# Kamino666/video_features

Hardware: AMD Instinct MI355X
Metric: frames/sec CLIP-ViT-B/32 uni_12 (higher is better)
Workload: dtype bf16; 1 GPU; model=CLIP-ViT-B/32, global_batch=256, seq_len=12, resolution=224, parallelism=dp1

## Files before the change

video_features_amd/models/clip_vit.py:

```python
from __future__ import annotations

from dataclasses import dataclass
from typing import Optional

import torch
import torch.nn.functional as F
from torch import nn

from .. import ops


@dataclass
class ViTConfig:
    input_resolution: int = 224
    patch_size: int = 32
    width: int = 768
    layers: int = 12
    heads: int = 12
    output_dim: int = 512


VIT_B32 = ViTConfig(patch_size=32)
VIT_B16 = ViTConfig(patch_size=16)

# ... 60 lines not shown
            ops.fused_ln_tiles(x, self.attn.proj.weight)
            and ops.fused_ln_tiles(x, self.mlp.c_fc.weight))

    def attn_mlp_folded(self, y1: torch.Tensor, s1: torch.Tensor):
        proj, fc, ln = self.attn.proj, self.mlp.c_fc, self.ln_2
        s2, st2 = ops.linear_res_stats(self.attn.heads_out(y1), proj.weight,
                                       proj.bias, s1)
        h = ops.linear_ln_act(
            s2, st2, *self._ln2_fold(), act='quick_gelu', eps=ln.eps,
            unfolded=(fc.weight, fc.bias, ln.weight, ln.bias))
        return self.mlp.c_proj(h), s2


class VisionTransformer(nn.Module):
    def __init__(self, cfg: ViTConfig = VIT_B32):
        super().__init__()
        self.cfg = cfg
        w = cfg.width
        self.conv1 = nn.Conv2d(3, w, kernel_size=cfg.patch_size,
                               stride=cfg.patch_size, bias=False)
        n_patches = (cfg.input_resolution // cfg.patch_size) ** 2
        scale = w ** -0.5
        self.class_embedding = nn.Parameter(scale * torch.randn(w))
        self.positional_embedding = nn.Parameter(
            scale * torch.randn(n_patches + 1, w))
        self.ln_pre = LayerNorm(w)
        self.blocks = nn.ModuleList(
            [ResidualAttentionBlock(w, cfg.heads) for _ in range(cfg.layers)])
        self.ln_post = LayerNorm(w)
        self.proj = nn.Parameter(scale * torch.randn(w, cfg.output_dim))

    def _patch_embed(self, x: torch.Tensor) -> torch.Tensor:
        if x.is_cuda:
            t = x.shape[0]
            p = self.cfg.patch_size
            g = x.shape[-1] // p
            xp = x.reshape(t, 3, g, p, g, p).permute(0, 2, 4, 1, 3, 5)
            xp = xp.reshape(t, g * g, 3 * p * p)
            w = self.conv1.weight.reshape(self.cfg.width, -1)
            return xp @ w.t()
        x = self.conv1(x)
        return x.flatten(2).transpose(1, 2)

    def forward(self, x: torch.Tensor) -> torch.Tensor:
        x = self._patch_embed(x)
        x = ops.clip_embed_ln(x, self.class_embedding,
                              self.positional_embedding, self.ln_pre.weight,
                              self.ln_pre.bias, self.ln_pre.eps)
        full_tail = ops._env_flag('VFA_CLIP_FULL_TAIL')
        delta, res = None, x
        for blk in (self.blocks if full_tail else self.blocks[:-1]):
            if delta is None:
                y1, s1 = blk.ln_1(res), res
            else:
                y1, s1 = ops.layer_norm_residual(delta, res, blk.ln_1.weight,
                                                 blk.ln_1.bias, blk.ln_1.eps)
            if blk.fold_routed(s1):
                delta, res = blk.attn_mlp_folded(y1, s1)
                continue
            a = blk.attn(y1)
            y2, s2 = ops.layer_norm_residual(a, s1, blk.ln_2.weight,
                                             blk.ln_2.bias, blk.ln_2.eps)
            delta, res = blk.mlp(y2), s2
        if full_tail:
            x = delta + res
            x = self.ln_post(x[:, 0, :])
        else:
            x = self._cls_tail(self.blocks[-1], delta, res)
        return x @ self.proj.to(x.dtype)

    def _cls_tail(self, blk: ResidualAttentionBlock,
# ... 31 lines not shown
```

video_features_amd/ops/__init__.py:

```python
from __future__ import annotations

import math
import os
from typing import Optional

import torch

_ext = None
_ext_err: Optional[str] = None


def _env_flag(name: str) -> bool:
    return os.environ.get(name, '').strip().lower() not in (
        '', '0', 'false', 'no', 'off')


def _load_extension():
    global _ext, _ext_err
    if _ext is not None or _ext_err is not None:
        return _ext
    try:
        from . import _vfa_hip
        _ext = _vfa_hip
    except ImportError as e:
# ... 95 lines not shown
        y, s = _ext.layer_norm_residual(x.contiguous(), res.contiguous(),
                                        weight, bias, eps)
        return y, s
    s = x + res
    y = torch.nn.functional.layer_norm(s, (s.shape[-1],), weight, bias, eps)
    return y, s


def clip_embed_ln(pe: torch.Tensor, cls: torch.Tensor, pos: torch.Tensor,
                  weight: torch.Tensor, bias: torch.Tensor,
                  eps: float = 1e-5) -> torch.Tensor:
    if (_use_hip(pe) and pe.shape[-1] % 8 == 0
            and pe.dtype in _FLOAT_DTYPES):
        return _ext.clip_embed_ln(pe.contiguous(), cls, pos, weight, bias,
                                  eps)
    c = cls.to(pe.dtype).expand(pe.shape[0], 1, -1)
    x = torch.cat([c, pe], dim=1) + pos.to(pe.dtype)
    return layer_norm(x, weight, bias, eps)


def preprocess_u8_chw(frames_u8: torch.Tensor, mean, std,
                      bf16: bool = True) -> torch.Tensor:
    if _use_hip(frames_u8) and \
            (frames_u8.shape[1] * frames_u8.shape[2]) % 4 == 0:
        return _ext.u8_chw_norm(frames_u8.contiguous(), list(map(float, mean)),
                                list(map(float, std)), bf16)
    x = frames_u8.permute(0, 3, 1, 2).float() / 255.0
    mean_t = torch.as_tensor(mean, dtype=x.dtype, device=x.device)
    std_t = torch.as_tensor(std, dtype=x.dtype, device=x.device)
    x = (x - mean_t[:, None, None]) / std_t[:, None, None]
    return x.to(torch.bfloat16) if bf16 else x


def mhsa_fused(qkv: torch.Tensor, heads: int,
               scale: Optional[float] = None) -> torch.Tensor:
    b, n, three_e = qkv.shape
    e = three_e // 3
    d = e // heads
    if scale is None:
        scale = 1.0 / math.sqrt(d)
    if _use_hip(qkv) and qkv.dtype == torch.bfloat16 and d == 64:
        qkv5 = qkv.view(b, n, 3, heads, d)
        return _ext.flash_qkv(qkv5.contiguous(), float(scale))
    q, k, v = qkv.view(b, n, 3, heads, d).permute(2, 0, 3, 1, 4).unbind(0)
    o = attention(q.contiguous(), k.contiguous(), v.contiguous(), scale)
    return o.permute(0, 2, 1, 3).reshape(b, n, e)


def pwc_correlation(f1: torch.Tensor, f2: torch.Tensor,
                    max_disp: int = 4, out: Optional[torch.Tensor] = None,
                    out_off: int = 0, act: str = 'none') -> torch.Tensor:
    if act not in ('none', 'leaky_relu'):
        raise ValueError(f'pwc_correlation: unsupported act {act!r}')
    leaky = act == 'leaky_relu'
    if _use_hip(f1):
        direct = out is None or (
            out.dtype == torch.bfloat16
            and out.is_contiguous(memory_format=torch.channels_last))
        if (max_disp == 4 and f1.dtype == torch.bfloat16
                and f2.dtype == torch.bfloat16 and _cl_only(f1)
                and _cl_only(f2)):
            y = _ext.pwc_correlation_nhwc(f1, f2, out if direct else None,
                                          out_off, leaky)
        else:
            y = _ext.pwc_correlation(f1.contiguous(), f2.contiguous(),
                                     max_disp, out if direct else None,
                                     out_off, leaky)
        if direct:
            return y
    else:
        y = _pwc_correlation_torch(f1, f2, max_disp)
        if leaky:
            y = torch.nn.functional.leaky_relu(y, 0.1)
    return _store_slice(out, out_off, y)


# ... 581 lines not shown
```

video_features_amd/ops/csrc/attention_flash.hip:

```cpp
#include "vfa_common.h"

typedef __bf16 bf16x8 __attribute__((ext_vector_type(8)));
typedef float f32x4 __attribute__((ext_vector_type(4)));

namespace {

constexpr int QBLK = 64;
constexpr int KVBLK = 64;
constexpr int D = 64;
constexpr int LSTR = D + 8;

__device__ __forceinline__ float group16_max(float v) {
#pragma unroll
  for (int off = 8; off > 0; off >>= 1) v = fmaxf(v, __shfl_xor(v, off, 64));
  return v;
}

__device__ __forceinline__ float group16_sum(float v) {
#pragma unroll
  for (int off = 8; off > 0; off >>= 1) v += __shfl_xor(v, off, 64);
  return v;
}

__device__ __forceinline__ void stage_rows(const __bf16* g, int rows,
// ... 137 lines not shown
      for (int r = 0; r < 4; ++r)
        p_lds[(hi4 * 4 + r) * LSTR + nt * 16 + lo] = (__bf16)p_vals[nt][r];
    asm volatile("s_waitcnt lgkmcnt(0)" ::: "memory");

#pragma unroll
    for (int kt = 0; kt < 2; ++kt) {
      bf16x8 a = *reinterpret_cast<const bf16x8*>(
          p_lds + lo * LSTR + kt * 32 + hi4 * 8);
#pragma unroll
      for (int nt = 0; nt < 4; ++nt) {
        bf16x8 bfr = *reinterpret_cast<const bf16x8*>(
            s_vt + (nt * 16 + lo) * LSTR + kt * 32 + hi4 * 8);
        o_acc[nt] =
            __builtin_amdgcn_mfma_f32_16x16x32_bf16(a, bfr, o_acc[nt], 0, 0, 0);
      }
    }
  }

#pragma unroll
  for (int r = 0; r < 4; ++r) {
    const int grow = qbase + wave * 16 + hi4 * 4 + r;
    if (grow >= n) continue;
    const float inv_l = 1.0f / l_run[r];
    __bf16* orow = out + ((long long)bi * n + grow) * (h_total * D) +
                   (long long)hi * D;
#pragma unroll
    for (int nt = 0; nt < 4; ++nt)
      orow[nt * 16 + lo] = (__bf16)(o_acc[nt][r] * inv_l);
  }
  __syncthreads();
  }
}

__global__ __launch_bounds__(256)
void flash_qkv_small_kernel(const __bf16* __restrict__ qkv,
                            __bf16* __restrict__ out,
                            int b_total, int n, int h_total, float scale) {
  extern __shared__ __attribute__((aligned(16))) char smem[];
  __bf16* s_k0 = reinterpret_cast<__bf16*>(smem);
  __bf16* s_vt0 = s_k0 + 2 * KVBLK * LSTR;
  __bf16* s_p = s_vt0 + 2 * D * LSTR;

  const int tid = threadIdx.x;
  const int lane = tid & 63, wave = tid >> 6;
  const int lo = lane & 15, hi4 = lane >> 4;
  const long long row_stride = 3LL * h_total * D;
  const int total = b_total * h_total;
  const int qr = min(wave * 16 + lo, n - 1);

  int bh = blockIdx.x;
  if (bh >= total) return;

  bf16x8 a_cur[2];
  {
    const int bi = bh / h_total, hi = bh % h_total;
    const __bf16* k_g = qkv + (long long)bi * n * row_stride +
                        ((long long)1 * h_total + hi) * D;
    stage_rows(k_g, KVBLK, row_stride, s_k0, n);
    stage_vt(k_g + (long long)h_total * D, row_stride, s_vt0, n);
    const __bf16* q_g = qkv + (long long)bi * n * row_stride +
                        (long long)hi * D;
#pragma unroll
    for (int kt = 0; kt < 2; ++kt)
      a_cur[kt] = *reinterpret_cast<const bf16x8*>(
          q_g + (long long)qr * row_stride + kt * 32 + hi4 * 8);
  }
  __syncthreads();

  int buf = 0;
  for (; bh < total; bh += gridDim.x) {
    const int nbh = bh + gridDim.x;
    const bool has_next = nbh < total;
    const int pf = has_next ? nbh : bh;
    const int pbi = pf / h_total, phi = pf % h_total;
    const __bf16* k_gn = qkv + (long long)pbi * n * row_stride +
                         ((long long)1 * h_total + phi) * D;
    const __bf16* v_gn = k_gn + (long long)h_total * D;
    uint4 kreg[2], vreg[2];
#pragma unroll
    for (int i = 0; i < 2; ++i) {
      const int t = tid + i * 256, row = t >> 3, seg = t & 7;
      kreg[i] = row < n ? *reinterpret_cast<const uint4*>(
                              k_gn + row * row_stride + seg * 8)
                        : uint4{0u, 0u, 0u, 0u};
    }
#pragma unroll
    for (int i = 0; i < 2; ++i) {
      const int t = tid + i * 256, key = t & 63, seg = t >> 6;
      vreg[i] = key < n ? *reinterpret_cast<const uint4*>(
                              v_gn + key * row_stride + seg * 8)
                        : uint4{0u, 0u, 0u, 0u};
    }
    bf16x8 a_next[2];
    {
      const __bf16* q_gn = qkv + (long long)pbi * n * row_stride +
                           (long long)phi * D;
#pragma unroll
      for (int kt = 0; kt < 2; ++kt)
        a_next[kt] = *reinterpret_cast<const bf16x8*>(
            q_gn + (long long)qr * row_stride + kt * 32 + hi4 * 8);
    }

    const __bf16* s_k = s_k0 + buf * KVBLK * LSTR;
    const __bf16* s_vt = s_vt0 + buf * D * LSTR;
    f32x4 s_frag[4];
#pragma unroll
    for (int t = 0; t < 4; ++t) s_frag[t] = f32x4{0.f, 0.f, 0.f, 0.f};
#pragma unroll
    for (int kt = 0; kt < 2; ++kt)
#pragma unroll
      for (int nt = 0; nt < 4; ++nt) {
        bf16x8 bfr = *reinterpret_cast<const bf16x8*>(
            s_k + (nt * 16 + lo) * LSTR + kt * 32 + hi4 * 8);
        s_frag[nt] = __builtin_amdgcn_mfma_f32_16x16x32_bf16(
            a_cur[kt], bfr, s_frag[nt], 0, 0, 0);
      }

    float p_vals[4][4], l_run[4];
#pragma unroll
    for (int r = 0; r < 4; ++r) {
      float mx = -1e30f;
#pragma unroll
      for (int nt = 0; nt < 4; ++nt) {
        float s = s_frag[nt][r] * scale;
        if (nt * 16 + lo >= n) s = -1e30f;
        s_frag[nt][r] = s;
        mx = fmaxf(mx, s);
      }
      mx = group16_max(mx);
      float rowsum = 0.f;
#pragma unroll
      for (int nt = 0; nt < 4; ++nt) {
        const float p = __expf(s_frag[nt][r] - mx);
        p_vals[nt][r] = p;
        rowsum += p;
      }
      l_run[r] = group16_sum(rowsum);
    }

    __bf16* p_lds = s_p + wave * 16 * LSTR;
#pragma unroll
    for (int nt = 0; nt < 4; ++nt)
#pragma unroll
      for (int r = 0; r < 4; ++r)
        p_lds[(hi4 * 4 + r) * LSTR + nt * 16 + lo] = (__bf16)p_vals[nt][r];
    asm volatile("s_waitcnt lgkmcnt(0)" ::: "memory");

    f32x4 o_acc[4];
#pragma unroll
    for (int t = 0; t < 4; ++t) o_acc[t] = f32x4{0.f, 0.f, 0.f, 0.f};
#pragma unroll
    for (int kt = 0; kt < 2; ++kt) {
      bf16x8 a = *reinterpret_cast<const bf16x8*>(
          p_lds + lo * LSTR + kt * 32 + hi4 * 8);
#pragma unroll
      for (int nt = 0; nt < 4; ++nt) {
        bf16x8 bfr = *reinterpret_cast<const bf16x8*>(
            s_vt + (nt * 16 + lo) * LSTR + kt * 32 + hi4 * 8);
        o_acc[nt] = __builtin_amdgcn_mfma_f32_16x16x32_bf16(
            a, bfr, o_acc[nt], 0, 0, 0);
      }
    }

    {
      const int bi = bh / h_total, hi = bh % h_total;
#pragma unroll
      for (int r = 0; r < 4; ++r) {
        const int grow = wave * 16 + hi4 * 4 + r;
        if (grow >= n) continue;
        const float inv_l = 1.0f / l_run[r];
        __bf16* orow = out + ((long long)bi * n + grow) * (h_total * D) +
                       (long long)hi * D;
#pragma unroll
        for (int nt = 0; nt < 4; ++nt)
          orow[nt * 16 + lo] = (__bf16)(o_acc[nt][r] * inv_l);
      }
    }

    __bf16* d_k = s_k0 + (buf ^ 1) * KVBLK * LSTR;
    __bf16* d_vt = s_vt0 + (buf ^ 1) * D * LSTR;
#pragma unroll
    for (int i = 0; i < 2; ++i) {
      const int t = tid + i * 256, row = t >> 3, seg = t & 7;
      *reinterpret_cast<uint4*>(d_k + row * LSTR + seg * 8) = kreg[i];
    }
#pragma unroll
    for (int i = 0; i < 2; ++i) {
      const int t = tid + i * 256, key = t & 63, seg = t >> 6;
      const __bf16* e = reinterpret_cast<const __bf16*>(&vreg[i]);
#pragma unroll
      for (int j = 0; j < 8; ++j) d_vt[(seg * 8 + j) * LSTR + key] = e[j];
    }
    __syncthreads();
    buf ^= 1;
    a_cur[0] = a_next[0];
    a_cur[1] = a_next[1];
  }
}

__global__ void mfma_gemm16_kernel(const float* a, const float* b, float* d) {
  const int l = threadIdx.x, lo = l & 15, hi4 = l >> 4;
  bf16x8 av, bv;
#pragma unroll
  for (int j = 0; j < 8; ++j) {
    av[j] = (__bf16)a[lo * 32 + hi4 * 8 + j];
    bv[j] = (__bf16)b[(hi4 * 8 + j) * 16 + lo];
  }
  f32x4 c = {0.f, 0.f, 0.f, 0.f};
  c = __builtin_amdgcn_mfma_f32_16x16x32_bf16(av, bv, c, 0, 0, 0);
#pragma unroll
  for (int r = 0; r < 4; ++r) d[(hi4 * 4 + r) * 16 + lo] = c[r];
}

}

extern "C" {

void vfa_flash_qkv(const void* qkv, void* out, int b, int n, int h,
                   float scale, hipStream_t stream) {
  static const bool no_pipe = [] {
    const char* e = getenv("VFA_NO_FLASHPIPE");
    return e && e[0] && e[0] != '0';
  }();
  if (n <= KVBLK && !no_pipe) {
    dim3 grid(min(b * h, 1024), 1);
    size_t lds = (size_t)(2 * (KVBLK + D) + 4 * 16) * LSTR * sizeof(__bf16);
    hipLaunchKernelGGL(flash_qkv_small_kernel, grid, dim3(256), lds, stream,
                       (const __bf16*)qkv, (__bf16*)out, b, n, h, scale);
    return;
  }
  dim3 grid(min(b * h, 2048), (n + QBLK - 1) / QBLK);
  size_t lds = (size_t)(QBLK + KVBLK + D + 4 * 16) * LSTR * sizeof(__bf16);
  hipLaunchKernelGGL(flash_qkv_kernel, grid, dim3(256), lds, stream,
                     (const __bf16*)qkv, (__bf16*)out, b, n, h, scale);
}

void vfa_mfma_gemm16(const void* a, const void* b, void* d,
                     hipStream_t stream) {
  hipLaunchKernelGGL(mfma_gemm16_kernel, dim3(1), dim3(64), 0, stream,
                     (const float*)a, (const float*)b, (float*)d);
}

}
```

video_features_amd/ops/csrc/attnpool.hip:

```cpp
#include "vfa_common.h"

namespace {

__global__ void attnpool_tokens_kernel(const uint4* __restrict__ x,
                                       const uint4* __restrict__ pos,
                                       uint4* __restrict__ t, long long b,
                                       int hw, int c8) {
  const long long total = b * c8;
  const float inv = 1.f / (float)hw;
  for (long long i = (long long)blockIdx.x * blockDim.x + threadIdx.x;
       i < total; i += (long long)gridDim.x * blockDim.x) {
    const long long bi = i / c8;
    const int ci = (int)(i % c8);
    const uint4* xb = x + bi * hw * c8 + ci;
    uint4* tb = t + bi * (hw + 1) * c8 + ci;
    float sum[8] = {0.f, 0.f, 0.f, 0.f, 0.f, 0.f, 0.f, 0.f};
    for (int j = 0; j < hw; ++j) {
      float xv[8], pv[8];
      bf16x8_to_f32(xb[(long long)j * c8], xv);
      bf16x8_to_f32(pos[(long long)(j + 1) * c8 + ci], pv);
#pragma unroll
      for (int e = 0; e < 8; ++e) {
        sum[e] += xv[e];
        xv[e] += pv[e];
      }
      tb[(long long)(j + 1) * c8] = f32_to_bf16x8(xv);
    }
    float pv[8];
    bf16x8_to_f32(pos[ci], pv);
#pragma unroll
    for (int e = 0; e < 8; ++e) sum[e] = sum[e] * inv + pv[e];
    tb[0] = f32_to_bf16x8(sum);
  }
}

__global__ __launch_bounds__(256) void attention_pool_d64_kernel(
    const __hip_bfloat16* __restrict__ q, const __hip_bfloat16* __restrict__ kv,
    __hip_bfloat16* __restrict__ out, long long bh, int heads, int l,
    float scale) {
  const int lane = threadIdx.x & 63;
  const long long pair = (long long)blockIdx.x * 4 + (threadIdx.x >> 6);
  if (pair >= bh) return;
  const long long bi = pair / heads;
  const int h = (int)(pair % heads);
  const long long c = (long long)heads * 64;
  float qf[64];
  {
    const uint4* qp = reinterpret_cast<const uint4*>(q + bi * c + h * 64);
#pragma unroll
    for (int s = 0; s < 8; ++s) {
      bf16x8_to_f32(qp[s], qf + 8 * s);
#pragma unroll
      for (int e = 0; e < 8; ++e) qf[8 * s + e] *= scale;
    }
  }
  const __hip_bfloat16* kb = kv + bi * l * 2 * c + h * 64;
  const __hip_bfloat16* vb = kb + c;
  float m = -INFINITY, denom = 0.f, acc = 0.f;
  for (int c0 = 0; c0 < l; c0 += 64) {
    const int nk = min(64, l - c0);
    const int j = c0 + lane;
    float s = -INFINITY;
    if (j < l) {
      const uint4* kp =
          reinterpret_cast<const uint4*>(kb + (long long)j * 2 * c);
      float dot = 0.f;
#pragma unroll
      for (int u = 0; u < 8; ++u) {
        float kf[8];
        bf16x8_to_f32(kp[u], kf);
#pragma unroll
        for (int e = 0; e < 8; ++e) dot += qf[8 * u + e] * kf[e];
      }
      s = dot;
    }
    const float m_new = fmaxf(m, wave_allreduce_max(s));
    const float p = (j < l) ? __expf(s - m_new) : 0.f;
    const float alpha = __expf(m - m_new);
    denom = denom * alpha + wave_allreduce_sum(p);
    acc *= alpha;
    const __hip_bfloat16* vp = vb + (long long)c0 * 2 * c + lane;
    for (int jj = 0; jj < nk; ++jj) {
      const float pj = __shfl(p, jj, 64);
      acc += pj * __bfloat162float(vp[(long long)jj * 2 * c]);
    }
    m = m_new;
  }
  out[bi * c + h * 64 + lane] = __float2bfloat16(acc / denom);
}

}

extern "C" {

void vfa_attnpool_tokens(const void* x, const void* pos, void* t, long long b,
                         int hw, int c, hipStream_t stream) {
  const long long total = b * (c / 8);
  if (total <= 0) return;
  const int grid = (int)min((total + 63) / 64, (long long)2048);
  hipLaunchKernelGGL(attnpool_tokens_kernel, dim3(grid), dim3(64), 0, stream,
                     (const uint4*)x, (const uint4*)pos, (uint4*)t, b, hw,
                     c / 8);
}

void vfa_attention_pool_d64(const void* q, const void* kv, void* out,
                            long long b, int heads, int l, float scale,
                            hipStream_t stream) {
  const long long bh = b * heads;
  if (bh <= 0) return;
  const long long grid = (bh + 3) / 4;
  hipLaunchKernelGGL(attention_pool_d64_kernel, dim3((unsigned)grid),
                     dim3(256), 0, stream, (const __hip_bfloat16*)q,
                     (const __hip_bfloat16*)kv, (__hip_bfloat16*)out, bh,
                     heads, l, scale);
}

}
```

video_features_amd/ops/csrc/bindings.cpp:

```cpp
#include <torch/extension.h>
#include <c10/hip/HIPStream.h>
#include <mutex>
#include <unordered_map>
#include <hip/hip_runtime.h>
#include <hip/hip_bf16.h>

#include "vfa_api.h"

namespace {

int dtype_tag(torch::ScalarType s) {
  switch (s) {
    case torch::kFloat32: return 0;
    case torch::kBFloat16: return 1;
    case torch::kFloat16: return 2;
    default:
      TORCH_CHECK(false, "unsupported dtype ", s);
  }
}

int dtype_tag(const torch::Tensor& t) { return dtype_tag(t.scalar_type()); }

hipStream_t current_stream() {
  return c10::hip::getCurrentHIPStream().stream();
// ... 211 lines not shown
                                               torch::Tensor b, double eps) {
  TORCH_CHECK(x.is_cuda() && x.is_contiguous() && res.is_contiguous());
  TORCH_CHECK(x.sizes() == res.sizes());
  const int d = (int)x.size(-1);
  auto wc = w.contiguous().to(x.scalar_type());
  auto bc = b.contiguous().to(x.scalar_type());
  auto y = torch::empty_like(x);
  auto s = torch::empty_like(x);
  vfa_layer_norm_residual(x.data_ptr(), res.data_ptr(), wc.data_ptr(),
                          bc.data_ptr(), y.data_ptr(), s.data_ptr(),
                          x.numel() / d, d, (float)eps, dtype_tag(x),
                          current_stream());
  return {y, s};
}

torch::Tensor u8_chw_norm(torch::Tensor frames, std::vector<double> mean,
                          std::vector<double> std_, bool bf16) {
  TORCH_CHECK(frames.is_cuda() && frames.is_contiguous());
  TORCH_CHECK(frames.scalar_type() == torch::kUInt8);
  TORCH_CHECK(frames.dim() == 4 && frames.size(3) == 3, "(T,H,W,3) expected");
  const long long t = frames.size(0);
  const int h = (int)frames.size(1), w = (int)frames.size(2);
  TORCH_CHECK((h * w) % 4 == 0);
  float m[3] = {(float)mean[0], (float)mean[1], (float)mean[2]};
  float s[3] = {(float)std_[0], (float)std_[1], (float)std_[2]};
  auto out = torch::empty({(long)t, 3, h, w},
                          frames.options().dtype(bf16 ? torch::kBFloat16
                                                      : torch::kFloat32));
  vfa_u8_chw_norm(frames.data_ptr(), out.data_ptr(), t, h, w, m, s,
                  bf16 ? 1 : 0, current_stream());
  return out;
}

torch::Tensor flash_qkv(torch::Tensor qkv, double scale) {
  TORCH_CHECK(qkv.is_cuda() && qkv.is_contiguous() && qkv.dim() == 5);
  TORCH_CHECK(qkv.size(2) == 3 && qkv.size(4) == 64,
              "flash_qkv covers head_dim 64");
  TORCH_CHECK(qkv.scalar_type() == torch::kBFloat16);
  const int b = (int)qkv.size(0), n = (int)qkv.size(1);
  const int h = (int)qkv.size(3);
  auto out = torch::empty({b, n, h * 64L}, qkv.options());
  vfa_flash_qkv(qkv.data_ptr(), out.data_ptr(), b, n, h, (float)scale,
                current_stream());
  return out;
}

torch::Tensor mfma_gemm16(torch::Tensor a, torch::Tensor b) {
  TORCH_CHECK(a.is_cuda() && a.is_contiguous() && b.is_contiguous());
  TORCH_CHECK(a.sizes() == torch::IntArrayRef({16, 32}) &&
              b.sizes() == torch::IntArrayRef({32, 16}));
  auto af = a.to(torch::kFloat32), bf = b.to(torch::kFloat32);
  auto d = torch::empty({16, 16}, af.options());
  vfa_mfma_gemm16(af.data_ptr(), bf.data_ptr(), d.data_ptr(),
                  current_stream());
  return d;
}

torch::Tensor corr_lookup(std::vector<torch::Tensor> pyramid,
                          torch::Tensor coords, bool nhwc,
                          torch::ScalarType out_dtype, bool force_gmem) {
  const int levels = (int)pyramid.size();
  TORCH_CHECK(levels >= 1 && levels <= 4, "1..4 pyramid levels");
  const int tag = dtype_tag(out_dtype);
  TORCH_CHECK(coords.is_cuda() && coords.dim() == 4 && coords.size(1) == 2);
  auto cc = coords.to(torch::kFloat32).contiguous();
  const long long b = coords.size(0);
  const int h = (int)coords.size(2), w = (int)coords.size(3);
  const long long npix = b * h * w;
  CorrPyramid pyr;
  long long lds_floats = 0;
  for (int l = 0; l < levels; ++l) {
    auto& t = pyramid[l];
    TORCH_CHECK(t.is_cuda() && t.is_contiguous() &&
                t.scalar_type() == torch::kFloat32);
    TORCH_CHECK(t.size(0) == npix && t.size(1) == 1, "plane-per-pixel");
    pyr.hs[l] = (int)t.size(2);
// ... 424 lines not shown
  auto t = torch::empty({x.size(0), hw + 1, c}, x.options());
  vfa_attnpool_tokens(x.data_ptr(), pos.data_ptr(), t.data_ptr(), x.size(0),
                      (int)hw, (int)c, current_stream());
  return t;
}

torch::Tensor attention_pool(torch::Tensor q, torch::Tensor kv,
                             int64_t heads) {
  TORCH_CHECK(q.is_cuda() && q.dim() == 2 && q.is_contiguous());
  TORCH_CHECK(kv.is_cuda() && kv.dim() == 3 && kv.is_contiguous());
  TORCH_CHECK(q.scalar_type() == torch::kBFloat16 &&
              kv.scalar_type() == torch::kBFloat16, "attention_pool: bf16");
  const int64_t b = q.size(0), c = q.size(1), l = kv.size(1);
  TORCH_CHECK(heads >= 1 && c == heads * 64,
              "attention_pool covers head_dim 64");
  TORCH_CHECK(kv.size(0) == b && kv.size(2) == 2 * c && l >= 1,
              "kv must be (B, L>=1, 2C)");
  auto out = torch::empty({b, c}, q.options());
  vfa_attention_pool_d64(q.data_ptr(), kv.data_ptr(), out.data_ptr(), b,
                         (int)heads, (int)l, 0.125f, current_stream());
  return out;
}

}

PYBIND11_MODULE(TORCH_EXTENSION_NAME, m) {
  m.def("quick_gelu", &quick_gelu);
  m.def("gelu_tanh", &gelu_tanh);
  m.def("layer_norm", &layer_norm);
  m.def("bilinear_warp", &bilinear_warp);
  m.def("grid_sample_bilinear", &grid_sample_bilinear);
  m.def("pwc_correlation", &pwc_correlation);
  m.def("mhsa", &mhsa);
  m.def("flash_qkv", &flash_qkv);
  m.def("mfma_gemm16", &mfma_gemm16);
  m.def("layer_norm_residual", &layer_norm_residual);
  m.def("clip_embed_ln", &clip_embed_ln);
  m.def("u8_chw_norm", &u8_chw_norm);
  m.def("corr_lookup", &corr_lookup);
  m.def("convex_upsample", &convex_upsample);
  m.def("gru_zr", &gru_zr);
  m.def("gru_out", &gru_out);
  m.def("instance_norm2d", &instance_norm2d);
  m.def("maxpool3d_same", &maxpool3d_same);
  m.def("maxpool2d_same", &maxpool2d_same);
  m.def("linear_act", &linear_act);
  m.def("linear_res_stats", &linear_res_stats);
  m.def("linear_ln_act", &linear_ln_act);
  m.def("conv2d_nhwc", &conv2d_nhwc);
  m.def("conv2d_tile", &conv2d_tile);
  m.def("conv_transpose2d_nhwc", &conv_transpose2d_nhwc);
  m.def("conv_transpose2d_small", &conv_transpose2d_small);
  m.def("bilinear_warp_nhwc", &bilinear_warp_nhwc);
  m.def("pwc_correlation_nhwc", &pwc_correlation_nhwc);
  m.def("temporal_merge", &temporal_merge);
  m.def("avgpool2d_nhwc", &avgpool2d_nhwc);
  m.def("attnpool_tokens", &attnpool_tokens);
  m.def("attention_pool", &attention_pool);
  m.attr("gfx_arch") = "gfx950";
}
```

video_features_amd/ops/csrc/preprocess.hip:

```cpp
#include "vfa_common.h"
#include <type_traits>

namespace {

template <typename T>
__global__ void u8_chw_norm_kernel(const unsigned char* __restrict__ in,
                                   T* __restrict__ out, long long t, int h,
                                   int w, float m0, float m1, float m2,
                                   float s0, float s1, float s2) {
  const long long hw = (long long)h * w;
  const long long quads_per_img = hw / 4;
  const long long total = t * quads_per_img;
  const float inv255 = 1.0f / 255.0f;
  const float im[3] = {m0, m1, m2};
  const float is[3] = {1.0f / s0, 1.0f / s1, 1.0f / s2};
  for (long long i = (long long)blockIdx.x * blockDim.x + threadIdx.x;
       i < total; i += (long long)gridDim.x * blockDim.x) {
    const long long ti = i / quads_per_img;
    const long long q = i % quads_per_img;
    const unsigned char* src = in + (ti * hw + q * 4) * 3;
    const uint3 raw = *reinterpret_cast<const uint3*>(src);
    unsigned char px[12];
    *reinterpret_cast<uint3*>(px) = raw;
    T planes[3][4];
#pragma unroll
    for (int p = 0; p < 4; ++p) {
#pragma unroll
      for (int c = 0; c < 3; ++c) {
        float v = (float)px[p * 3 + c] * inv255;
        planes[c][p] = from_f32<T>((v - im[c]) * is[c]);
      }
    }
    using VecElt =
        typename std::conditional<sizeof(T) == 2, unsigned short, unsigned>::type;
    using Vec = __attribute__((ext_vector_type(4))) VecElt;
#pragma unroll
    for (int c = 0; c < 3; ++c) {
      T* dst = out + (ti * 3 + c) * hw + q * 4;
      *reinterpret_cast<Vec*>(dst) = *reinterpret_cast<Vec*>(planes[c]);
    }
  }
}

}

extern "C" void vfa_u8_chw_norm(const void* in, void* out, long long t,
                                int h, int w, const float* mean,
                                const float* std, int dtype,
                                hipStream_t stream) {
  long long total = t * ((long long)h * w / 4);
  int block = 256;
  int grid = (int)min((total + block - 1) / block, (long long)4096);
  if (dtype == VFA_BF16) {
    hipLaunchKernelGGL((u8_chw_norm_kernel<__hip_bfloat16>), dim3(grid),
                       dim3(block), 0, stream, (const unsigned char*)in,
                       (__hip_bfloat16*)out, t, h, w, mean[0], mean[1],
                       mean[2], std[0], std[1], std[2]);
  } else {
    hipLaunchKernelGGL((u8_chw_norm_kernel<float>), dim3(grid), dim3(block),
                       0, stream, (const unsigned char*)in, (float*)out, t, h,
                       w, mean[0], mean[1], mean[2], std[0], std[1], std[2]);
  }
}
```

video_features_amd/ops/csrc/vfa_api.h:

```cpp
#pragma once
#include <hip/hip_runtime.h>

struct ConvGeom {
  int b, hp, wp, cin;
  int oh, ow, kout;
  int kh, kw, sh, sw;
  int pt, pl;
  int kr;
};

struct ConvAddr {
  int dh, dw;
  int ldx;
};

struct CorrPyramid {
  const void* lvl[4];
  int hs[4], ws[4];
};

struct PoolGeom {
  int in[3], out[3];
  int k[3], s[3];
  int pad[3];
// ... 21 lines not shown
void vfa_bilinear_warp(const void* x, const void* flow, void* out, int b,
                       int c, int h, int w, int dtype, hipStream_t stream);
void vfa_bilinear_warp_nhwc(const void* x, const void* flow, void* out, int b,
                            int c, int h, int w, long long fb, long long fc,
                            long long fh, long long fw, float scale,
                            hipStream_t stream);
void vfa_grid_sample(const void* x, const void* coords, void* out,
                     long long n, int c, int h, int w, int ho, int wo,
                     int dtype, hipStream_t stream);

void vfa_corr_repack(const void* in, void* out, int b, int c, int h, int w,
                     int dtype, hipStream_t stream);
void vfa_pwc_correlation(const void* f1, const void* f1p, const void* f2p,
                         void* out, int b, int c, int h, int w, int dtype,
                         int ldo, int leaky, hipStream_t stream);
void vfa_pwc_correlation_nhwc(const void* f1, const void* f2, void* out,
                              int b, int c, int h, int w, int ldo, int leaky,
                              hipStream_t stream);

long long vfa_tconv_lds_bytes(int c, int kout);
void vfa_tconv_pform(const void* x, const void* wp, const void* bias,
                     void* part, void* out, int b, int h, int w, int c,
                     int ldx, int kout, int ldo, hipStream_t stream);
void vfa_tconv_direct(const void* x, const void* wgt, const void* bias,
                      void* out, int b, int c, int h, int w, long long sb,
                      long long sc, long long sh, long long sw, int kout,
                      int ldo, hipStream_t stream);

void vfa_mhsa_small(const void* q, const void* k, const void* v, void* out,
                    int bh, int n, int d, float scale, int dtype,
                    hipStream_t stream);

void vfa_flash_qkv(const void* qkv, void* out, int b, int n, int h,
                   float scale, hipStream_t stream);
void vfa_mfma_gemm16(const void* a, const void* b, void* d,
                     hipStream_t stream);

void vfa_u8_chw_norm(const void* in, void* out, long long t, int h, int w,
                     const float* mean, const float* std, int dtype,
                     hipStream_t stream);

void vfa_corr_lookup(const CorrPyramid& pyr, const void* coords, void* out,
                     int levels, long long npix, int hw, int lds_floats,
                     int nhwc, int dtype, hipStream_t stream);
void vfa_convex_upsample(const void* flow, const void* mask, void* out, int b,
                         int h, int w, int nhwc, int dtype,
                         hipStream_t stream);
void vfa_gru_zr(const void* zr, const void* hx, void* rhx, void* z, int b,
                int c, int cx, long long hw, int nhwc, int dtype,
                hipStream_t stream);
void vfa_gru_out(const void* q, const void* z, void* hx, int b, int c, int cx,
                 long long hw, int nhwc, int dtype, hipStream_t stream);

void vfa_instance_norm2d(const void* x, void* out, int b, int c, int hw,
                         float eps, int relu, int nhwc, int dtype,
                         hipStream_t stream);

void vfa_maxpool3d_same(const void* x, void* out, long long bc,
                        const PoolGeom& g, int dtype, hipStream_t stream);
void vfa_maxpool2d_same(const void* x, void* out, long long n, int c,
                        const PoolGeom& g, int nhwc, int dtype,
                        hipStream_t stream);
void vfa_avgpool2d_nhwc(const void* x, void* out, long long n, int c, int ih,
                        int iw, int oh, int ow, int k, hipStream_t stream);

void vfa_linear_act(const void* a, const void* w, const void* bias,
                    const void* res, void* c, int m, int n, int k, int act,
                    hipStream_t stream);
void vfa_linear_res_stats(const void* a, const void* w, const void* bias,
                          const void* res, void* c, void* part, int m, int n,
                          int k, hipStream_t stream);
void vfa_linear_ln_act(const void* a, const void* stats, int groups,
                       const void* w, const void* ln_c, const void* ln_b,
// ... 24 lines not shown
```

Baseline: 87150 frames/sec.

## Rewrite small-seq flash attention with register-resident 32x32 MFMA, add patchify kernel

Replaces the block-per-head small-sequence attention kernel with a wave-per-(head, 32-query block) kernel. It keeps Q and K in registers, uses 32x32x16 MFMAs, and reads V through a transposing LDS load (ds_read_b64_tr_b16). Softmax reductions use permlane32 swaps, and the next unit's loads are prefetched in software. It also adds a dedicated vectorized patchify kernel in place of the torch permute+copy, and rewrites the attention-pool kernel to process 8 keys per wave iteration with vectorized K/V loads. The aim is to remove LDS round-trips, __syncthreads, and the extra permute copy, at the cost of more complex register-heavy code that depends on gfx950-specific instructions.

Result: faster. 90050 frames/sec, median of 6 (+3.3%).

```diff
diff --git a/video_features_amd/models/clip_vit.py b/video_features_amd/models/clip_vit.py
--- a/video_features_amd/models/clip_vit.py
+++ b/video_features_amd/models/clip_vit.py
@@ -116,11 +116,7 @@
 
     def _patch_embed(self, x: torch.Tensor) -> torch.Tensor:
         if x.is_cuda:
-            t = x.shape[0]
-            p = self.cfg.patch_size
-            g = x.shape[-1] // p
-            xp = x.reshape(t, 3, g, p, g, p).permute(0, 2, 4, 1, 3, 5)
-            xp = xp.reshape(t, g * g, 3 * p * p)
+            xp = ops.patchify(x, self.cfg.patch_size)
             w = self.conv1.weight.reshape(self.cfg.width, -1)
             return xp @ w.t()
         x = self.conv1(x)
diff --git a/video_features_amd/ops/__init__.py b/video_features_amd/ops/__init__.py
--- a/video_features_amd/ops/__init__.py
+++ b/video_features_amd/ops/__init__.py
@@ -151,8 +151,29 @@
     return x.to(torch.bfloat16) if bf16 else x
 
 
+def patchify(x: torch.Tensor, p: int) -> torch.Tensor:
+    t, c, h, w = x.shape
+    if h % p or w % p:
+        raise ValueError(f'patchify: H, W = {h}, {w} must be multiples of '
+                         f'p = {p}')
+    es = x.element_size()
+    if (_use_hip(x) and es in (2, 4) and (p * es) % 16 == 0
+            and x.numel() > 0):
+        xc = x.contiguous()
+        if xc.data_ptr() % 16 == 0:
+            return _ext.patchify(xc, int(p))
+    gy, gx = h // p, w // p
+    xp = x.reshape(t, c, gy, p, gx, p).permute(0, 2, 4, 1, 3, 5)
+    return xp.reshape(t, gy * gx, c * p * p)
+
+
+MHSA_VARIANTS = (0, 1)
+
+
 def mhsa_fused(qkv: torch.Tensor, heads: int,
-               scale: Optional[float] = None) -> torch.Tensor:
+               scale: Optional[float] = None, variant: int = 0) -> torch.Tensor:
+    if variant not in MHSA_VARIANTS:
+        raise ValueError(f'mhsa_fused: variant must be one of {MHSA_VARIANTS}')
     b, n, three_e = qkv.shape
     e = three_e // 3
     d = e // heads
@@ -160,7 +181,7 @@
         scale = 1.0 / math.sqrt(d)
     if _use_hip(qkv) and qkv.dtype == torch.bfloat16 and d == 64:
         qkv5 = qkv.view(b, n, 3, heads, d)
-        return _ext.flash_qkv(qkv5.contiguous(), float(scale))
+        return _ext.flash_qkv(qkv5.contiguous(), float(scale), int(variant))
     q, k, v = qkv.view(b, n, 3, heads, d).permute(2, 0, 3, 1, 4).unbind(0)
     o = attention(q.contiguous(), k.contiguous(), v.contiguous(), scale)
     return o.permute(0, 2, 1, 3).reshape(b, n, e)
diff --git a/video_features_amd/ops/csrc/attention_flash.hip b/video_features_amd/ops/csrc/attention_flash.hip
--- a/video_features_amd/ops/csrc/attention_flash.hip
+++ b/video_features_amd/ops/csrc/attention_flash.hip
@@ -193,169 +193,187 @@
   }
 }
 
-__global__ __launch_bounds__(256)
-void flash_qkv_small_kernel(const __bf16* __restrict__ qkv,
-                            __bf16* __restrict__ out,
-                            int b_total, int n, int h_total, float scale) {
-  extern __shared__ __attribute__((aligned(16))) char smem[];
-  __bf16* s_k0 = reinterpret_cast<__bf16*>(smem);
-  __bf16* s_vt0 = s_k0 + 2 * KVBLK * LSTR;
-  __bf16* s_p = s_vt0 + 2 * D * LSTR;
-
-  const int tid = threadIdx.x;
-  const int lane = tid & 63, wave = tid >> 6;
-  const int lo = lane & 15, hi4 = lane >> 4;
+typedef float f32x16 __attribute__((ext_vector_type(16)));
+typedef unsigned u32x2 __attribute__((ext_vector_type(2)));
+
+constexpr int RSTR = 192;
+constexpr int RIMG = 64 * RSTR;
+constexpr int RWAVES = 4;
+constexpr int RBLOCKS = 768;
+
+struct RegsLoads {
+  bf16x8 k[2][4];
+  bf16x8 q[4];
+  uint4 v[8];
+};
+
+__device__ __forceinline__ void regs_load(RegsLoads& ld,
+                                          const __bf16* __restrict__ qkv,
+                                          int u, int nqb, int n, int h_total,
+                                          int lane) {
+  const int pair = u / nqb, qb = u - pair * nqb;
+  const int bi = pair / h_total, hi = pair - bi * h_total;
   const long long row_stride = 3LL * h_total * D;
-  const int total = b_total * h_total;
-  const int qr = min(wave * 16 + lo, n - 1);
-
-  int bh = blockIdx.x;
-  if (bh >= total) return;
-
-  bf16x8 a_cur[2];
-  {
-    const int bi = bh / h_total, hi = bh % h_total;
-    const __bf16* k_g = qkv + (long long)bi * n * row_stride +
-                        ((long long)1 * h_total + hi) * D;
-    stage_rows(k_g, KVBLK, row_stride, s_k0, n);
-    stage_vt(k_g + (long long)h_total * D, row_stride, s_vt0, n);
-    const __bf16* q_g = qkv + (long long)bi * n * row_stride +
-                        (long long)hi * D;
+  const __bf16* base = qkv + (long long)bi * n * row_stride + (long long)hi * D;
+  const int r = lane & 31, h8 = (lane >> 5) * 8;
+  const __bf16* qp = base + (long long)min(qb * 32 + r, n - 1) * row_stride + h8;
+#pragma unroll
+  for (int s = 0; s < 4; ++s)
+    ld.q[s] = *reinterpret_cast<const bf16x8*>(qp + s * 16);
+#pragma unroll
+  for (int kt = 0; kt < 2; ++kt) {
+    const __bf16* kp = base + (long long)h_total * D +
+                       (long long)min(kt * 32 + r, n - 1) * row_stride + h8;
+#pragma unroll
+    for (int s = 0; s < 4; ++s)
+      ld.k[kt][s] = *reinterpret_cast<const bf16x8*>(kp + s * 16);
+  }
+  const __bf16* vp = base + 2LL * h_total * D + (lane & 7) * 8;
+#pragma unroll
+  for (int i = 0; i < 8; ++i)
+    ld.v[i] = *reinterpret_cast<const uint4*>(
+        vp + (long long)min(i * 8 + (lane >> 3), n - 1) * row_stride);
+}
+
+#define VFA_TR8(OFF)                                            \
+  asm volatile(                                                 \
+      "ds_read_b64_tr_b16 %0, %8 offset:" #OFF "+0\n\t"         \
+      "ds_read_b64_tr_b16 %1, %8 offset:" #OFF "+1536\n\t"      \
+      "ds_read_b64_tr_b16 %2, %8 offset:" #OFF "+3072\n\t"      \
+      "ds_read_b64_tr_b16 %3, %8 offset:" #OFF "+4608\n\t"      \
+      "ds_read_b64_tr_b16 %4, %8 offset:" #OFF "+6144\n\t"      \
+      "ds_read_b64_tr_b16 %5, %8 offset:" #OFF "+7680\n\t"      \
+      "ds_read_b64_tr_b16 %6, %8 offset:" #OFF "+9216\n\t"      \
+      "ds_read_b64_tr_b16 %7, %8 offset:" #OFF "+10752\n\t"     \
+      "s_waitcnt lgkmcnt(0)"                                    \
+      : "=&v"(t[0]), "=&v"(t[1]), "=&v"(t[2]), "=&v"(t[3]),     \
+        "=&v"(t[4]), "=&v"(t[5]), "=&v"(t[6]), "=&v"(t[7])      \
+      : "v"(tr_addr)                                            \
+      : "memory")
+
+__device__ __forceinline__ bf16x8 regs_join(u32x2 lo, u32x2 hi) {
+  typedef unsigned u32x4 __attribute__((ext_vector_type(4)));
+  const u32x4 v = {lo[0], lo[1], hi[0], hi[1]};
+  return __builtin_bit_cast(bf16x8, v);
+}
+
+__global__ __launch_bounds__(RWAVES * 64)
+__attribute__((amdgpu_waves_per_eu(3, 3)))
+void flash_qkv_regs_kernel(const __bf16* __restrict__ qkv,
+                           __bf16* __restrict__ out,
+                           int units, int nqb, int n, int h_total,
+                           float scale) {
+  __shared__ __attribute__((aligned(16))) char s_v[RWAVES * RIMG];
+  const int lane = threadIdx.x & 63;
+  const int wave = __builtin_amdgcn_readfirstlane(threadIdx.x >> 6);
+  const int nwaves = gridDim.x * RWAVES;
+  int u = blockIdx.x * RWAVES + wave;
+  if (u >= units) return;
+  char* img = s_v + wave * RIMG;
+  const int r = lane & 31, h = lane >> 5;
+  char* st_addr = img + (lane >> 3) * RSTR + (lane & 7) * 16;
+  const unsigned tr_addr =
+      (unsigned)(size_t)img +
+      (((lane & 15) >> 2) + 4 * h) * RSTR + (16 * ((lane >> 4) & 1) + 4 * (lane & 3)) * 2;
+
+  RegsLoads cur;
+  regs_load(cur, qkv, u, nqb, n, h_total, lane);
+  for (; u < units; u += nwaves) {
+#pragma unroll
+    for (int i = 0; i < 8; ++i)
+      *reinterpret_cast<uint4*>(st_addr + i * 8 * RSTR) = cur.v[i];
+
+    f32x16 st[2];
+#pragma unroll
+    for (int kt = 0; kt < 2; ++kt) {
+#pragma unroll
+      for (int e = 0; e < 16; ++e) st[kt][e] = 0.f;
+#pragma unroll
+      for (int s = 0; s < 4; ++s)
+        st[kt] = __builtin_amdgcn_mfma_f32_32x32x16_bf16(cur.k[kt][s], cur.q[s],
+                                                         st[kt], 0, 0, 0);
+    }
+
+    const int un = (u + nwaves < units) ? u + nwaves : u;
+    RegsLoads nxt;
+    regs_load(nxt, qkv, un, nqb, n, h_total, lane);
+
+    float mx = -INFINITY;
+    int nl = n - 4 * h;
+    asm volatile("" : "+v"(nl));
 #pragma unroll
     for (int kt = 0; kt < 2; ++kt)
-      a_cur[kt] = *reinterpret_cast<const bf16x8*>(
-          q_g + (long long)qr * row_stride + kt * 32 + hi4 * 8);
-  }
-  __syncthreads();
-
-  int buf = 0;
-  for (; bh < total; bh += gridDim.x) {
-    const int nbh = bh + gridDim.x;
-    const bool has_next = nbh < total;
-    const int pf = has_next ? nbh : bh;
-    const int pbi = pf / h_total, phi = pf % h_total;
-    const __bf16* k_gn = qkv + (long long)pbi * n * row_stride +
-                         ((long long)1 * h_total + phi) * D;
-    const __bf16* v_gn = k_gn + (long long)h_total * D;
-    uint4 kreg[2], vreg[2];
-#pragma unroll
-    for (int i = 0; i < 2; ++i) {
-      const int t = tid + i * 256, row = t >> 3, seg = t & 7;
-      kreg[i] = row < n ? *reinterpret_cast<const uint4*>(
-                              k_gn + row * row_stride + seg * 8)
-                        : uint4{0u, 0u, 0u, 0u};
-    }
-#pragma unroll
-    for (int i = 0; i < 2; ++i) {
-      const int t = tid + i * 256, key = t & 63, seg = t >> 6;
-      vreg[i] = key < n ? *reinterpret_cast<const uint4*>(
-                              v_gn + key * row_stride + seg * 8)
-                        : uint4{0u, 0u, 0u, 0u};
-    }
-    bf16x8 a_next[2];
+#pragma unroll
+      for (int e = 0; e < 16; ++e) {
+        const int key = 32 * kt + (e & 3) + 8 * (e >> 2);
+        const float s = key < nl ? st[kt][e] * scale : -INFINITY;
+        st[kt][e] = s;
+        mx = fmaxf(mx, s);
+      }
     {
-      const __bf16* q_gn = qkv + (long long)pbi * n * row_stride +
-                           (long long)phi * D;
+      const unsigned b = __float_as_uint(mx);
+      const u32x2 sw = __builtin_amdgcn_permlane32_swap(b, b, false, false);
+      mx = fmaxf(__uint_as_float(sw[0]), __uint_as_float(sw[1]));
+    }
+    float l = 0.f;
+    bf16x8 pf[2][2];
+#pragma unroll
+    for (int kt = 0; kt < 2; ++kt)
+#pragma unroll
+      for (int e = 0; e < 16; ++e) {
+        const float p = __expf(st[kt][e] - mx);
+        l += p;
+        pf[kt][e >> 3][e & 7] = (__bf16)p;
+      }
+    {
+      const unsigned b = __float_as_uint(l);
+      const u32x2 sw = __builtin_amdgcn_permlane32_swap(b, b, false, false);
+      l = __uint_as_float(sw[0]) + __uint_as_float(sw[1]);
+    }
+    const float inv_l = 1.0f / l;
+
+    const int pair = u / nqb, qb = u - pair * nqb;
+    const int bi = pair / h_total, hi = pair - bi * h_total;
+    const int qrow = qb * 32 + r;
+    __bf16* orow = out + ((long long)bi * n + min(qrow, n - 1)) * (h_total * D) +
+                   (long long)hi * D + 8 * h;
+#pragma unroll
+    for (int dt = 0; dt < 2; ++dt) {
+      u32x2 t[8];
+      if (dt == 0) VFA_TR8(0); else VFA_TR8(64);
+      f32x16 o;
+#pragma unroll
+      for (int e = 0; e < 16; ++e) o[e] = 0.f;
 #pragma unroll
       for (int kt = 0; kt < 2; ++kt)
-        a_next[kt] = *reinterpret_cast<const bf16x8*>(
-            q_gn + (long long)qr * row_stride + kt * 32 + hi4 * 8);
-    }
-
-    const __bf16* s_k = s_k0 + buf * KVBLK * LSTR;
-    const __bf16* s_vt = s_vt0 + buf * D * LSTR;
-    f32x4 s_frag[4];
-#pragma unroll
-    for (int t = 0; t < 4; ++t) s_frag[t] = f32x4{0.f, 0.f, 0.f, 0.f};
-#pragma unroll
-    for (int kt = 0; kt < 2; ++kt)
-#pragma unroll
-      for (int nt = 0; nt < 4; ++nt) {
-        bf16x8 bfr = *reinterpret_cast<const bf16x8*>(
-            s_k + (nt * 16 + lo) * LSTR + kt * 32 + hi4 * 8);
-        s_frag[nt] = __builtin_amdgcn_mfma_f32_16x16x32_bf16(
-            a_cur[kt], bfr, s_frag[nt], 0, 0, 0);
-      }
-
-    float p_vals[4][4], l_run[4];
-#pragma unroll
-    for (int r = 0; r < 4; ++r) {
-      float mx = -1e30f;
-#pragma unroll
-      for (int nt = 0; nt < 4; ++nt) {
-        float s = s_frag[nt][r] * scale;
-        if (nt * 16 + lo >= n) s = -1e30f;
-        s_frag[nt][r] = s;
-        mx = fmaxf(mx, s);
-      }
-      mx = group16_max(mx);
-      float rowsum = 0.f;
-#pragma unroll
-      for (int nt = 0; nt < 4; ++nt) {
-        const float p = __expf(s_frag[nt][r] - mx);
-        p_vals[nt][r] = p;
-        rowsum += p;
-      }
-      l_run[r] = group16_sum(rowsum);
-    }
-
-    __bf16* p_lds = s_p + wave * 16 * LSTR;
-#pragma unroll
-    for (int nt = 0; nt < 4; ++nt)
-#pragma unroll
-      for (int r = 0; r < 4; ++r)
-        p_lds[(hi4 * 4 + r) * LSTR + nt * 16 + lo] = (__bf16)p_vals[nt][r];
-    asm volatile("s_waitcnt lgkmcnt(0)" ::: "memory");
-
-    f32x4 o_acc[4];
-#pragma unroll
-    for (int t = 0; t < 4; ++t) o_acc[t] = f32x4{0.f, 0.f, 0.f, 0.f};
-#pragma unroll
-    for (int kt = 0; kt < 2; ++kt) {
-      bf16x8 a = *reinterpret_cast<const bf16x8*>(
-          p_lds + lo * LSTR + kt * 32 + hi4 * 8);
-#pragma unroll
-      for (int nt = 0; nt < 4; ++nt) {
-        bf16x8 bfr = *reinterpret_cast<const bf16x8*>(
-            s_vt + (nt * 16 + lo) * LSTR + kt * 32 + hi4 * 8);
-        o_acc[nt] = __builtin_amdgcn_mfma_f32_16x16x32_bf16(
-            a, bfr, o_acc[nt], 0, 0, 0);
-      }
-    }
-
-    {
-      const int bi = bh / h_total, hi = bh % h_total;
-#pragma unroll
-      for (int r = 0; r < 4; ++r) {
-        const int grow = wave * 16 + hi4 * 4 + r;
-        if (grow >= n) continue;
-        const float inv_l = 1.0f / l_run[r];
-        __bf16* orow = out + ((long long)bi * n + grow) * (h_total * D) +
-                       (long long)hi * D;
-#pragma unroll
-        for (int nt = 0; nt < 4; ++nt)
-          orow[nt * 16 + lo] = (__bf16)(o_acc[nt][r] * inv_l);
-      }
-    }
-
-    __bf16* d_k = s_k0 + (buf ^ 1) * KVBLK * LSTR;
-    __bf16* d_vt = s_vt0 + (buf ^ 1) * D * LSTR;
-#pragma unroll
-    for (int i = 0; i < 2; ++i) {
-      const int t = tid + i * 256, row = t >> 3, seg = t & 7;
-      *reinterpret_cast<uint4*>(d_k + row * LSTR + seg * 8) = kreg[i];
-    }
-#pragma unroll
-    for (int i = 0; i < 2; ++i) {
-      const int t = tid + i * 256, key = t & 63, seg = t >> 6;
-      const __bf16* e = reinterpret_cast<const __bf16*>(&vreg[i]);
-#pragma unroll
-      for (int j = 0; j < 8; ++j) d_vt[(seg * 8 + j) * LSTR + key] = e[j];
-    }
-    __syncthreads();
-    buf ^= 1;
-    a_cur[0] = a_next[0];
-    a_cur[1] = a_next[1];
+#pragma unroll
+        for (int s = 0; s < 2; ++s)
+          o = __builtin_amdgcn_mfma_f32_32x32x16_bf16(
+              regs_join(t[4 * kt + 2 * s], t[4 * kt + 2 * s + 1]), pf[kt][s],
+              o, 0, 0, 0);
+      typedef __bf16 bf16x4 __attribute__((ext_vector_type(4)));
+      uint4 w[2];
+#pragma unroll
+      for (int g = 0; g < 4; g += 2) {
+        bf16x4 a, b;
+#pragma unroll
+        for (int e = 0; e < 4; ++e) {
+          a[e] = (__bf16)(o[4 * g + e] * inv_l);
+          b[e] = (__bf16)(o[4 * g + 4 + e] * inv_l);
+        }
+        const u32x2 ua = __builtin_bit_cast(u32x2, a);
+        const u32x2 ub = __builtin_bit_cast(u32x2, b);
+        const u32x2 x = __builtin_amdgcn_permlane32_swap(ua[0], ub[0], false, false);
+        const u32x2 y = __builtin_amdgcn_permlane32_swap(ua[1], ub[1], false, false);
+        w[g >> 1] = uint4{x[0], y[0], x[1], y[1]};
+      }
+      if (qrow < n) {
+#pragma unroll
+        for (int g = 0; g < 2; ++g)
+          *reinterpret_cast<uint4*>(orow + 32 * dt + 16 * g) = w[g];
+      }
+    }
+    cur = nxt;
   }
 }
 
@@ -378,16 +396,15 @@
 extern "C" {
 
 void vfa_flash_qkv(const void* qkv, void* out, int b, int n, int h,
-                   float scale, hipStream_t stream) {
-  static const bool no_pipe = [] {
-    const char* e = getenv("VFA_NO_FLASHPIPE");
-    return e && e[0] && e[0] != '0';
-  }();
-  if (n <= KVBLK && !no_pipe) {
-    dim3 grid(min(b * h, 1024), 1);
-    size_t lds = (size_t)(2 * (KVBLK + D) + 4 * 16) * LSTR * sizeof(__bf16);
-    hipLaunchKernelGGL(flash_qkv_small_kernel, grid, dim3(256), lds, stream,
-                       (const __bf16*)qkv, (__bf16*)out, b, n, h, scale);
+                   float scale, int variant, hipStream_t stream) {
+  if ((long long)b * h <= 0 || n <= 0) return;
+  if (n <= KVBLK && variant == 0) {
+    const int nqb = (n + 31) / 32;
+    const int units = b * h * nqb;
+    dim3 grid(min((units + RWAVES - 1) / RWAVES, RBLOCKS));
+    hipLaunchKernelGGL(flash_qkv_regs_kernel, grid, dim3(RWAVES * 64), 0,
+                       stream, (const __bf16*)qkv, (__bf16*)out, units, nqb,
+                       n, h, scale);
     return;
   }
   dim3 grid(min(b * h, 2048), (n + QBLK - 1) / QBLK);
diff --git a/video_features_amd/ops/csrc/attnpool.hip b/video_features_amd/ops/csrc/attnpool.hip
--- a/video_features_amd/ops/csrc/attnpool.hip
+++ b/video_features_amd/ops/csrc/attnpool.hip
@@ -39,54 +39,78 @@
     __hip_bfloat16* __restrict__ out, long long bh, int heads, int l,
     float scale) {
   const int lane = threadIdx.x & 63;
+  const int g = lane >> 3, sg = lane & 7;
   const long long pair = (long long)blockIdx.x * 4 + (threadIdx.x >> 6);
   if (pair >= bh) return;
   const long long bi = pair / heads;
   const int h = (int)(pair % heads);
   const long long c = (long long)heads * 64;
-  float qf[64];
-  {
-    const uint4* qp = reinterpret_cast<const uint4*>(q + bi * c + h * 64);
+  float qf[8];
+  bf16x8_to_f32(
+      *reinterpret_cast<const uint4*>(q + bi * c + h * 64 + sg * 8), qf);
 #pragma unroll
-    for (int s = 0; s < 8; ++s) {
-      bf16x8_to_f32(qp[s], qf + 8 * s);
+  for (int e = 0; e < 8; ++e) qf[e] *= scale;
+  const __hip_bfloat16* kb = kv + bi * l * 2 * c + h * 64 + sg * 8;
+  float m = -INFINITY, denom = 0.f;
+  float acc[8] = {0.f, 0.f, 0.f, 0.f, 0.f, 0.f, 0.f, 0.f};
+  for (int c0 = 0; c0 < l; c0 += 64) {
+    uint4 kr[8], vr[8];
 #pragma unroll
-      for (int e = 0; e < 8; ++e) qf[8 * s + e] *= scale;
+    for (int r = 0; r < 8; ++r) {
+      const int j = c0 + 8 * r + g;
+      kr[r] = vr[r] = uint4{0u, 0u, 0u, 0u};
+      if (j < l) {
+        const __hip_bfloat16* kp = kb + (long long)j * 2 * c;
+        kr[r] = *reinterpret_cast<const uint4*>(kp);
+        vr[r] = *reinterpret_cast<const uint4*>(kp + c);
+      }
     }
-  }
-  const __hip_bfloat16* kb = kv + bi * l * 2 * c + h * 64;
-  const __hip_bfloat16* vb = kb + c;
-  float m = -INFINITY, denom = 0.f, acc = 0.f;
-  for (int c0 = 0; c0 < l; c0 += 64) {
-    const int nk = min(64, l - c0);
-    const int j = c0 + lane;
-    float s = -INFINITY;
-    if (j < l) {
-      const uint4* kp =
-          reinterpret_cast<const uint4*>(kb + (long long)j * 2 * c);
+    float s[8];
+    float mx = -INFINITY;
+#pragma unroll
+    for (int r = 0; r < 8; ++r) {
+      float kf[8];
+      bf16x8_to_f32(kr[r], kf);
       float dot = 0.f;
 #pragma unroll
-      for (int u = 0; u < 8; ++u) {
-        float kf[8];
-        bf16x8_to_f32(kp[u], kf);
+      for (int e = 0; e < 8; ++e) dot += qf[e] * kf[e];
 #pragma unroll
-        for (int e = 0; e < 8; ++e) dot += qf[8 * u + e] * kf[e];
-      }
-      s = dot;
+      for (int off = 1; off < 8; off <<= 1) dot += __shfl_xor(dot, off, 64);
+      s[r] = (c0 + 8 * r + g < l) ? dot : -INFINITY;
+      mx = fmaxf(mx, s[r]);
     }
-    const float m_new = fmaxf(m, wave_allreduce_max(s));
-    const float p = (j < l) ? __expf(s - m_new) : 0.f;
+#pragma unroll
+    for (int off = 8; off < 64; off <<= 1)
+      mx = fmaxf(mx, __shfl_xor(mx, off, 64));
+    const float m_new = fmaxf(m, mx);
     const float alpha = __expf(m - m_new);
-    denom = denom * alpha + wave_allreduce_sum(p);
-    acc *= alpha;
-    const __hip_bfloat16* vp = vb + (long long)c0 * 2 * c + lane;
-    for (int jj = 0; jj < nk; ++jj) {
-      const float pj = __shfl(p, jj, 64);
-      acc += pj * __bfloat162float(vp[(long long)jj * 2 * c]);
+    float psum = 0.f;
+#pragma unroll
+    for (int e = 0; e < 8; ++e) acc[e] *= alpha;
+#pragma unroll
+    for (int r = 0; r < 8; ++r) {
+      const float p = __expf(s[r] - m_new);
+      psum += p;
+      float vf[8];
+      bf16x8_to_f32(vr[r], vf);
+#pragma unroll
+      for (int e = 0; e < 8; ++e) acc[e] += p * vf[e];
     }
+#pragma unroll
+    for (int off = 8; off < 64; off <<= 1) psum += __shfl_xor(psum, off, 64);
+    denom = denom * alpha + psum;
     m = m_new;
   }
-  out[bi * c + h * 64 + lane] = __float2bfloat16(acc / denom);
+#pragma unroll
+  for (int e = 0; e < 8; ++e) {
+#pragma unroll
+    for (int off = 8; off < 64; off <<= 1)
+      acc[e] += __shfl_xor(acc[e], off, 64);
+    acc[e] /= denom;
+  }
+  if (g == 0)
+    *reinterpret_cast<uint4*>(out + bi * c + h * 64 + sg * 8) =
+        f32_to_bf16x8(acc);
 }
 
 }
diff --git a/video_features_amd/ops/csrc/bindings.cpp b/video_features_amd/ops/csrc/bindings.cpp
--- a/video_features_amd/ops/csrc/bindings.cpp
+++ b/video_features_amd/ops/csrc/bindings.cpp
@@ -267,7 +267,26 @@
   return out;
 }
 
-torch::Tensor flash_qkv(torch::Tensor qkv, double scale) {
+torch::Tensor patchify(torch::Tensor x, int64_t p) {
+  TORCH_CHECK(x.is_cuda() && x.is_contiguous() && x.dim() == 4,
+              "patchify: contiguous (T, C, H, W) expected");
+  const int64_t es = x.element_size();
+  const int64_t t = x.size(0), c = x.size(1), h = x.size(2), w = x.size(3);
+  TORCH_CHECK((es == 2 || es == 4) && p > 0 && (p * es) % 16 == 0 &&
+              h % p == 0 && w % p == 0,
+              "patchify: itemsize 2 or 4, p * itemsize % 16 == 0 and "
+              "H, W multiples of p required");
+  TORCH_CHECK(c * h * w * es / 16 < (1LL << 31), "patchify: frame too large");
+  auto out = torch::empty({t, (h / p) * (w / p), c * p * p}, x.options());
+  TORCH_CHECK((uintptr_t)x.data_ptr() % 16 == 0 &&
+              (uintptr_t)out.data_ptr() % 16 == 0,
+              "patchify: 16-B aligned tensors required");
+  vfa_patchify(x.data_ptr(), out.data_ptr(), t, (int)c, (int)h, (int)w,
+               (int)p, (int)es, current_stream());
+  return out;
+}
+
+torch::Tensor flash_qkv(torch::Tensor qkv, double scale, int64_t variant) {
   TORCH_CHECK(qkv.is_cuda() && qkv.is_contiguous() && qkv.dim() == 5);
   TORCH_CHECK(qkv.size(2) == 3 && qkv.size(4) == 64,
               "flash_qkv covers head_dim 64");
@@ -275,8 +294,10 @@
   const int b = (int)qkv.size(0), n = (int)qkv.size(1);
   const int h = (int)qkv.size(3);
   auto out = torch::empty({b, n, h * 64L}, qkv.options());
+  TORCH_CHECK(variant == 0 || variant == 1, "flash_qkv: variant 0 or 1");
+  TORCH_CHECK((int64_t)b * h * 2 < (1LL << 31), "flash_qkv: too many pairs");
   vfa_flash_qkv(qkv.data_ptr(), out.data_ptr(), b, n, h, (float)scale,
-                current_stream());
+                (int)variant, current_stream());
   return out;
 }
 
@@ -767,11 +788,13 @@
   m.def("grid_sample_bilinear", &grid_sample_bilinear);
   m.def("pwc_correlation", &pwc_correlation);
   m.def("mhsa", &mhsa);
-  m.def("flash_qkv", &flash_qkv);
+  m.def("flash_qkv", &flash_qkv, py::arg("qkv"), py::arg("scale"),
+        py::arg("variant") = 0);
   m.def("mfma_gemm16", &mfma_gemm16);
   m.def("layer_norm_residual", &layer_norm_residual);
   m.def("clip_embed_ln", &clip_embed_ln);
   m.def("u8_chw_norm", &u8_chw_norm);
+  m.def("patchify", &patchify);
   m.def("corr_lookup", &corr_lookup);
   m.def("convex_upsample", &convex_upsample);
   m.def("gru_zr", &gru_zr);
diff --git a/video_features_amd/ops/csrc/preprocess.hip b/video_features_amd/ops/csrc/preprocess.hip
--- a/video_features_amd/ops/csrc/preprocess.hip
+++ b/video_features_amd/ops/csrc/preprocess.hip
@@ -42,6 +42,51 @@
   }
 }
 
+__global__ __launch_bounds__(256) void patchify_kernel(
+    const uint4* __restrict__ in, uint4* __restrict__ out, int t, unsigned c,
+    unsigned h, unsigned p, unsigned gx, unsigned segs,
+    unsigned frame_units) {
+  const unsigned u = blockIdx.x * 256u + threadIdx.x;
+  if (u >= frame_units) return;
+  const unsigned seg = u % segs;
+  unsigned r = u / segs;
+  const unsigned py = r % p;
+  r /= p;
+  const unsigned ci = r % c;
+  r /= c;
+  const unsigned gxi = r % gx, gyi = r / gx;
+  const unsigned src =
+      (ci * h + gyi * p + py) * (gx * segs) + gxi * segs + seg;
+  const uint4* ip = in + src;
+  uint4* op = out + u;
+  const long long fs = frame_units;
+  const int step = gridDim.y;
+  int ti = blockIdx.y;
+  for (; ti + 3 * step < t; ti += 4 * step) {
+    uint4 v[4];
+#pragma unroll
+    for (int i = 0; i < 4; ++i) v[i] = ip[(ti + (long long)i * step) * fs];
+#pragma unroll
+    for (int i = 0; i < 4; ++i) op[(ti + (long long)i * step) * fs] = v[i];
+  }
+  for (; ti < t; ti += step) op[ti * fs] = ip[ti * fs];
+}
+
+}
+
+extern "C" void vfa_patchify(const void* in, void* out, long long t, int c,
+                             int h, int w, int p, int itemsize,
+                             hipStream_t stream) {
+  const int v = 16 / itemsize;
+  const long long frame_units = (long long)c * h * w / v;
+  if (t <= 0 || frame_units <= 0) return;
+  const unsigned bx = (unsigned)((frame_units + 255) / 256);
+  const long long want = (4096 + bx - 1) / bx;
+  const unsigned by = (unsigned)max(1LL, min(min(t, want), 65535LL));
+  hipLaunchKernelGGL(patchify_kernel, dim3(bx, by), dim3(256), 0, stream,
+                     (const uint4*)in, (uint4*)out, (int)t, (unsigned)c,
+                     (unsigned)h, (unsigned)p, (unsigned)(w / p),
+                     (unsigned)(p / v), (unsigned)frame_units);
 }
 
 extern "C" void vfa_u8_chw_norm(const void* in, void* out, long long t,
diff --git a/video_features_amd/ops/csrc/vfa_api.h b/video_features_amd/ops/csrc/vfa_api.h
--- a/video_features_amd/ops/csrc/vfa_api.h
+++ b/video_features_amd/ops/csrc/vfa_api.h
@@ -77,13 +77,15 @@
                     hipStream_t stream);
 
 void vfa_flash_qkv(const void* qkv, void* out, int b, int n, int h,
-                   float scale, hipStream_t stream);
+                   float scale, int variant, hipStream_t stream);
 void vfa_mfma_gemm16(const void* a, const void* b, void* d,
                      hipStream_t stream);
 
 void vfa_u8_chw_norm(const void* in, void* out, long long t, int h, int w,
                      const float* mean, const float* std, int dtype,
                      hipStream_t stream);
+void vfa_patchify(const void* in, void* out, long long t, int c, int h, int w,
+                  int p, int itemsize, hipStream_t stream);
 
 void vfa_corr_lookup(const CorrPyramid& pyr, const void* coords, void* out,
                      int levels, long long npix, int hw, int lds_floats,
```
